# evan-wes/nerf-sandbox

Hardware: NVIDIA B200
Metric: train_rays_per_s (higher is better)
Workload: dtype bf16

## Files before the change

nerf_sandbox_b200/csrc/field_tc.cu:

```cuda
#include <cuda.h>
#include <cuda_bf16.h>
#include <cuda_fp16.h>
#include <cstdio>
#include <mutex>
#include "nsb_common.cuh"
#include "tc_ptx.cuh"

namespace nsb {
namespace tc {

constexpr int TILE_M = 128;
constexpr int kStageBytes = 16384;
constexpr int kStages = 4;
constexpr int kActBytes = TILE_M * 256 * 2;
constexpr int kGxBytes = TILE_M * 64 * 2;
constexpr int kSmemAct = 0;
constexpr int kSmemGx = 2 * kActBytes;
constexpr int kSmemRing = kSmemGx + 2 * kGxBytes;
constexpr int kSmemBar = kSmemRing + kStages * kStageBytes;
constexpr int kSmemBias = kSmemBar + 256;
constexpr int kSmemBytes = kSmemBias + 2048;
constexpr int kThreads = 384;
constexpr int kStages2 = 8;
constexpr int kStageBytes2 = kStageBytes / 2;
static_assert(8 * (3 * kStages2 + 6) + 4 <= 256, "barrier block overflow");
constexpr int kNumMmaLayers = 10;
constexpr uint32_t kTmemCols = 512;

__constant__ uint32_t c_layer_ofs[kNumMmaLayers] = {0,      32768,  163840, 294912, 425984,
                                                    589824, 720896, 851968, 983040, 1114112};
constexpr uint32_t kWeightImageBytes = 1114112 + 288 * 128 * 2;
constexpr uint32_t kBiasOfs = kWeightImageBytes;
constexpr int kBiasFloats = 9 * 256 + 128;
constexpr int kWsigOfs = kBiasFloats;
constexpr int kBsigOfs = kWsigOfs + 256;
constexpr int kWoOfs = kBsigOfs + 4;
constexpr int kBoOfs = kWoOfs + 384;
constexpr int kTailFloats = kBoOfs + 4;
constexpr uint32_t kTImgOfs = ((kBiasOfs + kTailFloats * 4 + 255) / 256) * 256;
constexpr int kNumDgradLayers = 9;
__host__ __device__ inline uint32_t dgrad_layer_ofs(int m) { return kTImgOfs + (m == 0 ? 0u : 65536u + (uint32_t)(m - 1) * 131072u); }
constexpr uint32_t kF16ImgOfs = kTImgOfs + 65536 + 8 * 131072;
static_assert(kF16ImgOfs % 256 == 0 && kWeightImageBytes % 256 == 0, "images are addressed as rows of 256 B");
constexpr uint32_t kF16LoImgOfs = kF16ImgOfs + kWeightImageBytes;
constexpr uint32_t kDinImgOfs = kF16LoImgOfs + kWeightImageBytes;
constexpr uint32_t kDinPos0 = 0, kDinPos4 = 32768, kDinDir = 65536, kDinImgBytes = 73728;
constexpr uint32_t kPackedTcBytes = kDinImgOfs + kDinImgBytes;

__host__ __device__ inline int layer_nslabs(int l) { return l == 0 ? 2 : (l == 4 ? 10 : (l == 9 ? 9 : 8)); }
__host__ __device__ inline int layer_N(int l) { return l == 9 ? 128 : 256; }
__host__ __device__ inline int layer_bias_ofs(int l) { return l * 256; }

constexpr uint32_t kFmtF16 = 0u, kFmtBF16 = 1u;
__device__ __forceinline__ uint32_t make_idesc2(int N, uint32_t a_fmt, uint32_t b_fmt) {
    return (1u << 4) | (a_fmt << 7) | (b_fmt << 10) | ((uint32_t)(N >> 3) << 17) | ((uint32_t)((2 * TILE_M) >> 4) << 24);
}

__device__ __forceinline__ uint32_t pack_bf16_relu(float a, float b) {
    uint32_t d;
    asm("cvt.rn.relu.bf16x2.f32 %0, %1, %2;" : "=r"(d) : "f"(b), "f"(a));
    return d;
}
__device__ __forceinline__ uint32_t pack_bf16(float a, float b) {
    __nv_bfloat162 t = __floats2bfloat162_rn(a, b);
    return *reinterpret_cast<uint32_t*>(&t);
}
__device__ __forceinline__ uint32_t pack_f16(float a, float b) {
    uint32_t d;
    asm("cvt.rn.satfinite.f16x2.f32 %0, %1, %2;" : "=r"(d) : "f"(b), "f"(a));
    return d;
}
__device__ __forceinline__ uint32_t pack_f16_relu(float a, float b) {
    uint32_t d;
    asm("cvt.rn.relu.satfinite.f16x2.f32 %0, %1, %2;" : "=r"(d) : "f"(b), "f"(a));
    return d;
}
template <bool F16> __device__ __forceinline__ uint32_t pack2(float a, float b) { return F16 ? pack_f16(a, b) : pack_bf16(a, b); }
template <bool F16> __device__ __forceinline__ uint32_t pack2_relu(float a, float b) { return F16 ? pack_f16_relu(a, b) : pack_bf16_relu(a, b); }

__device__ __forceinline__ uint32_t relu_bits16(const uint32_t (&w)[8]) {
    uint32_t s = 0;
#pragma unroll
    for (int j = 0; j < 8; ++j) s += __vsetne2(w[j], 0u) << j;
    return s;
}
__device__ __forceinline__ uint32_t relu_mask_word(uint32_t bits16, int j) { return ((bits16 >> j) & 0x00010001u) * 0xFFFFu; }

__device__ __forceinline__ void st_chunk(uint32_t base, int k8, int r, uint32_t a, uint32_t b, uint32_t c, uint32_t d);
__device__ __forceinline__ void st_chunk_g(uint8_t* grow, int k8, uint32_t a, uint32_t b, uint32_t c, uint32_t d);
__device__ __forceinline__ float4 lds_f4(uint32_t addr) {
    float4 v;
    asm volatile("ld.shared.v4.f32 {%0, %1, %2, %3}, [%4];" : "=f"(v.x), "=f"(v.y), "=f"(v.z), "=f"(v.w) : "r"(addr));
    return v;
}
template <int KIND, bool MASK>
__device__ __forceinline__ void epi_chunk16(const uint32_t (&v)[16], int c0, const float4 (&bias)[4], uint32_t act, int r, float& sig,
                                            float (&rgb)[3], float hw0, float hw1, float hw2, uint32_t& mbits) {
    float f[16];
#pragma unroll
    for (int j = 0; j < 4; ++j) {
        f[4 * j] = __uint_as_float(v[4 * j]) + bias[j].x; f[4 * j + 1] = __uint_as_float(v[4 * j + 1]) + bias[j].y;
        f[4 * j + 2] = __uint_as_float(v[4 * j + 2]) + bias[j].z; f[4 * j + 3] = __uint_as_float(v[4 * j + 3]) + bias[j].w;
    }
    if (KIND == 1 || KIND == 3) {
// ... 8 lines not shown
                rgb[2] = fmaf(f[j], __shfl_sync(0xffffffffu, hw2, src0 + j), rgb[2]);
            }
        }
    }
    if (KIND != 3 || MASK) {
        uint32_t w[8];
#pragma unroll
        for (int j = 0; j < 8; ++j) w[j] = KIND == 0 ? pack2_relu<!MASK>(f[2 * j], f[2 * j + 1]) : pack2<!MASK>(f[2 * j], f[2 * j + 1]);
        st_chunk(act, (c0 >> 3), r, w[0], w[1], w[2], w[3]);
        st_chunk(act, (c0 >> 3) + 1, r, w[4], w[5], w[6], w[7]);
        if (KIND != 2 && MASK) mbits = relu_bits16(w);
    }
}
template <int KIND, bool MASK>
__device__ __forceinline__ void epi_columns(uint32_t tmem_row, uint32_t sbias, uint32_t act, int r, int lane, const float* __restrict__ tail,
                                            float& sig, float (&rgb)[3], uint32_t* gmask) {
    constexpr int N = KIND == 3 ? 128 : 256;
    float hw0 = 0.f, hw1 = 0.f, hw2 = 0.f;
    if (KIND == 1) hw0 = __ldg(tail + kWsigOfs + lane);
    if (KIND == 3) { hw0 = __ldg(tail + kWoOfs + lane); hw1 = __ldg(tail + kWoOfs + 128 + lane); hw2 = __ldg(tail + kWoOfs + 256 + lane); }
    uint32_t mw[8] = {0u, 0u, 0u, 0u, 0u, 0u, 0u, 0u};
    uint32_t va[16], vb[16];
    tc_ld16(tmem_row, va);
#pragma unroll 1
    for (int c0 = 0; c0 < N; c0 += 32) {
        float4 ba[4], bb[4];
#pragma unroll
        for (int j = 0; j < 4; ++j) { ba[j] = lds_f4(sbias + 4u * (uint32_t)(c0 + 4 * j)); bb[j] = lds_f4(sbias + 4u * (uint32_t)(c0 + 16 + 4 * j)); }
        float n0 = 0.f, n1 = 0.f, n2 = 0.f;
        if (KIND == 1 && c0 + 32 < N) n0 = __ldg(tail + kWsigOfs + c0 + 32 + lane);
        if (KIND == 3 && c0 + 32 < N) {
            n0 = __ldg(tail + kWoOfs + c0 + 32 + lane); n1 = __ldg(tail + kWoOfs + 128 + c0 + 32 + lane);
            n2 = __ldg(tail + kWoOfs + 256 + c0 + 32 + lane);
        }
        tc_wait_ld();
        tc_ld16(tmem_row + (uint32_t)c0 + 16u, vb);
        pin16(va);
        uint32_t m0 = 0, m1 = 0;
        epi_chunk16<KIND, MASK>(va, c0, ba, act, r, sig, rgb, hw0, hw1, hw2, m0);
        tc_wait_ld();
        tc_ld16(tmem_row + (uint32_t)(c0 + 32 < N ? c0 + 32 : c0), va);
        pin16(vb);
        epi_chunk16<KIND, MASK>(vb, c0 + 16, bb, act, r, sig, rgb, hw0, hw1, hw2, m1);
        if (MASK) {
            const uint32_t m = m0 | (m1 << 8);
#pragma unroll
            for (int k = 0; k < 8; ++k) mw[k] = (c0 >> 5) == k ? m : mw[k];
        }
        hw0 = n0; hw1 = n1; hw2 = n2;
    }
    if (MASK && gmask) {
        reinterpret_cast<uint4*>(gmask)[0] = make_uint4(mw[0], mw[1], mw[2], mw[3]);
        reinterpret_cast<uint4*>(gmask)[1] = make_uint4(mw[4], mw[5], mw[6], mw[7]);
    }
}

struct FwdParams {
    const float* rays_o; const float* rays_d; const float* z; const float* ray_norm; const float* viewdirs;
    const float* enc_pos; const float* enc_dir;
    const uint8_t* packed;
    float* raw;
    uint8_t* stash;
    float* dbg; int dbg_layer;
    unsigned long long* cyc;
    int64_t Q; int N;
    int64_t num_tiles;
    alignas(64) CUtensorMap tm8;
    alignas(64) CUtensorMap tm4;
};

constexpr size_t kStashGx = 0, kStashH = 16384, kStashFeat = kStashH + 8 * 65536, kStashGd = kStashFeat + 65536,
                 kStashC = kStashGd + 8192,
                 kStashMask = kStashC + 32768, kStashTile = kStashMask + 9 * 128 * 32;
constexpr size_t kDstashTile = 32768 + 9 * 65536;
__host__ __device__ inline size_t dstash_ofs(int k) { return k == 9 ? 0 : 32768 + (size_t)(8 - k) * 65536; }

__device__ __forceinline__ void named_bar_sync(int id, int nthreads) {
    asm volatile("bar.sync %0, %1;" ::"r"(id), "r"(nthreads) : "memory");
}
__device__ __forceinline__ void named_bar_arrive(int id, int nthreads) {
    asm volatile("bar.arrive %0, %1;" ::"r"(id), "r"(nthreads) : "memory");
}
constexpr int kHandoffBar = 3;
__device__ __forceinline__ void handoff_signal(int t) {
    tc_fence_before();
    named_bar_arrive(kHandoffBar + t, 160);
}
__device__ __forceinline__ void handoff_wait(int t) {
    named_bar_sync(kHandoffBar + t, 160);
    tc_fence_after();
    fence_async_smem();
    tc_fence_before();
}
__device__ __forceinline__ void arrive_in(uint32_t crank, uint32_t bar_in, uint32_t bar_pin, int t) {
    if (crank == 0) mbar_arrive(bar_in + 8 * t); else mbar_arrive_remote(bar_pin + 8 * t, 0);
}
__device__ __forceinline__ void bulk_wait_all0() { asm volatile("cp.async.bulk.wait_group 0;" ::: "memory"); }

__device__ __forceinline__ void st_chunk(uint32_t base, int k8, int r, uint32_t a, uint32_t b, uint32_t c, uint32_t d) {
    asm volatile("st.shared.v4.b32 [%0], {%1, %2, %3, %4};" ::"r"(base + (uint32_t)k8 * 2048u + (uint32_t)r * 16u), "r"(a), "r"(b),
                 "r"(c), "r"(d)
                 : "memory");
}

__device__ __forceinline__ void st_chunk_g(uint8_t* grow, int k8, uint32_t a, uint32_t b, uint32_t c, uint32_t d) {
    if (grow) *reinterpret_cast<uint4*>(grow + (size_t)k8 * 2048) = make_uint4(a, b, c, d);
}

template <bool F16>
__device__ __forceinline__ void encode_pos(uint32_t gx, int r, float px, float py, float pz, uint8_t* grow) {
    float e[64];
    e[0] = px; e[1] = py; e[2] = pz; e[63] = 0.f;
    float s[3], c[3];
    sincosf(px, &s[0], &c[0]); sincosf(py, &s[1], &c[1]); sincosf(pz, &s[2], &c[2]);
#pragma unroll
    for (int k = 0; k < 10; ++k) {
#pragma unroll
        for (int d = 0; d < 3; ++d) {
            e[3 + 3 * k + d] = s[d]; e[33 + 3 * k + d] = c[d];
            const float s2 = 2.0f * s[d] * c[d], c2 = fmaf(-2.0f * s[d], s[d], 1.0f);
            s[d] = s2; c[d] = c2;
        }
    }
#pragma unroll
    for (int k8 = 0; k8 < 8; ++k8) {
        const uint32_t w0 = pack2<F16>(e[8 * k8], e[8 * k8 + 1]), w1 = pack2<F16>(e[8 * k8 + 2], e[8 * k8 + 3]),
                       w2 = pack2<F16>(e[8 * k8 + 4], e[8 * k8 + 5]), w3 = pack2<F16>(e[8 * k8 + 6], e[8 * k8 + 7]);
        st_chunk(gx, k8, r, w0, w1, w2, w3);
        st_chunk_g(grow, k8, w0, w1, w2, w3);
    }
}
template <bool F16>
__device__ __forceinline__ void encode_dir(uint32_t gx, int r, float vx, float vy, float vz, uint8_t* grow) {
    float e[32];
#pragma unroll
    for (int i = 27; i < 32; ++i) e[i] = 0.f;
    e[0] = vx; e[1] = vy; e[2] = vz;
    float s[3], c[3];
    sincosf(vx, &s[0], &c[0]); sincosf(vy, &s[1], &c[1]); sincosf(vz, &s[2], &c[2]);
#pragma unroll
    for (int k = 0; k < 4; ++k) {
#pragma unroll
        for (int d = 0; d < 3; ++d) {
            e[3 + 3 * k + d] = s[d]; e[15 + 3 * k + d] = c[d];
            const float s2 = 2.0f * s[d] * c[d], c2 = fmaf(-2.0f * s[d], s[d], 1.0f);
            s[d] = s2; c[d] = c2;
        }
    }
#pragma unroll
    for (int k8 = 0; k8 < 4; ++k8) {
        const uint32_t w0 = pack2<F16>(e[8 * k8], e[8 * k8 + 1]), w1 = pack2<F16>(e[8 * k8 + 2], e[8 * k8 + 3]),
                       w2 = pack2<F16>(e[8 * k8 + 4], e[8 * k8 + 5]), w3 = pack2<F16>(e[8 * k8 + 6], e[8 * k8 + 7]);
        st_chunk(gx, k8, r, w0, w1, w2, w3);
        st_chunk_g(grow, k8, w0, w1, w2, w3);
    }
}
template <bool F16>
__device__ __forceinline__ void copy_enc_row(uint32_t gx, int r, const float* __restrict__ src, int n, int chunks, uint8_t* grow) {
    for (int k8 = 0; k8 < chunks; ++k8) {
        float v[8];
#pragma unroll
        for (int j = 0; j < 8; ++j) v[j] = (8 * k8 + j < n && src) ? src[8 * k8 + j] : 0.f;
        const uint32_t w0 = pack2<F16>(v[0], v[1]), w1 = pack2<F16>(v[2], v[3]), w2 = pack2<F16>(v[4], v[5]), w3 = pack2<F16>(v[6], v[7]);
        st_chunk(gx, k8, r, w0, w1, w2, w3);
        st_chunk_g(grow, k8, w0, w1, w2, w3);
    }
// ... 531 lines not shown
    }
    tc_fence_before();
    __syncthreads();
    cluster_sync_all();
    if (warp == 2) {
        tc_fence_after();
        asm volatile("tcgen05.dealloc.cta_group::2.sync.aligned.b32 %0, %1;" ::"r"(tmem_base), "r"(kTmemCols) : "memory");
    }
}

__device__ __forceinline__ float f16_residual(float x) {
    const __half h = __float2half_rn(fminf(fmaxf(x, -65504.0f), 65504.0f));
    return (x - __half2float(h)) * 2048.0f;
}
template <int FMT>
__device__ __forceinline__ void pack_tc_forward(const float* __restrict__ params, uint8_t* __restrict__ out, int m) {
    constexpr bool F16 = FMT != 0;
    {
        const int pl = m < 9 ? m : 10;
        const LayerDesc d = layer_desc(pl);
        const int N = d.N, Kp = d.Kpad;
        __nv_bfloat16* img = reinterpret_cast<__nv_bfloat16*>(out + (FMT == 2 ? kF16LoImgOfs : FMT == 1 ? kF16ImgOfs : 0u) + c_layer_ofs[m]);
        const int hn = N >> 1;
        for (int idx = blockIdx.x * blockDim.x + threadIdx.x; idx < N * (Kp >> 3); idx += gridDim.x * blockDim.x) {
            const int k8 = idx / N, n = idx % N;
            const float* row = params + d.w_off + (int64_t)n * d.K + 8 * k8;
            uint32_t w[4];
#pragma unroll
            for (int j = 0; j < 4; ++j) {
                float a = 8 * k8 + 2 * j < d.K ? row[2 * j] : 0.f, b = 8 * k8 + 2 * j + 1 < d.K ? row[2 * j + 1] : 0.f;
                if (FMT == 2) { a = f16_residual(a); b = f16_residual(b); }
                w[j] = pack2<F16>(a, b);
            }
            reinterpret_cast<uint4*>(img)[(((size_t)(k8 >> 2) * 2 + n / hn) * 4 + (k8 & 3)) * hn + n % hn] = make_uint4(w[0], w[1], w[2], w[3]);
        }
        if (FMT != 0) return;
        float* tail = reinterpret_cast<float*>(out + kBiasOfs);
        for (int n = blockIdx.x * blockDim.x + threadIdx.x; n < N; n += gridDim.x * blockDim.x)
            tail[layer_bias_ofs(m) + n] = params[d.b_off + n];
    }
    if (m == 0) {
        float* tail = reinterpret_cast<float*>(out + kBiasOfs);
        const LayerDesc ds = layer_desc(9), dc = layer_desc(11);
        for (int i = blockIdx.x * blockDim.x + threadIdx.x; i < 256; i += gridDim.x * blockDim.x) tail[kWsigOfs + i] = params[ds.w_off + i];
        for (int i = blockIdx.x * blockDim.x + threadIdx.x; i < 384; i += gridDim.x * blockDim.x) tail[kWoOfs + i] = params[dc.w_off + i];
        if (blockIdx.x == 0 && threadIdx.x < 4) {
            tail[kBsigOfs + threadIdx.x] = threadIdx.x == 0 ? params[ds.b_off] : 0.f;
            tail[kBoOfs + threadIdx.x] = threadIdx.x < 3 ? params[dc.b_off + threadIdx.x] : 0.f;
        }
    }
}

struct DgradParams {
    const float* d_raw;
    const uint8_t* packed;
    const uint8_t* stash;
    uint8_t* dstash;
    int64_t Q; int64_t num_tiles;
    alignas(64) CUtensorMap tm8;
};

__device__ __forceinline__ uint4 ldg16(const uint8_t* p) { return __ldg(reinterpret_cast<const uint4*>(p)); }
__device__ __forceinline__ float bf16lo(uint32_t w) { return __uint_as_float(w << 16); }
__device__ __forceinline__ float bf16hi(uint32_t w) { return __uint_as_float(w & 0xffff0000u); }

template <int KIND>
__device__ __forceinline__ void dgrad_chunk16(const uint32_t (&v)[16], int c0, uint32_t act, int r, float dsig, float hw0, uint32_t bits16) {
    uint32_t w[8];
#pragma unroll
    for (int j = 0; j < 8; ++j) {
        float a = __uint_as_float(v[2 * j]), b = __uint_as_float(v[2 * j + 1]);
        if (KIND == 1) {
            a = fmaf(dsig, __shfl_sync(0xffffffffu, hw0, (c0 & 16) + 2 * j), a);
            b = fmaf(dsig, __shfl_sync(0xffffffffu, hw0, (c0 & 16) + 2 * j + 1), b);
        }
        w[j] = pack_bf16(a, b);
        if (KIND != 0) w[j] &= relu_mask_word(bits16, j);
    }
    st_chunk(act, (c0 >> 3), r, w[0], w[1], w[2], w[3]);
    st_chunk(act, (c0 >> 3) + 1, r, w[4], w[5], w[6], w[7]);
}
template <int KIND>
__device__ __forceinline__ void dgrad_columns(uint32_t tmem_row, uint32_t act, int r, int lane, const float* __restrict__ tail,
                                              const uint4& mlo, const uint4& mhi, float dsig) {
    float hw0 = KIND == 1 ? __ldg(tail + kWsigOfs + lane) : 0.f;
    const uint32_t mw[8] = {mlo.x, mlo.y, mlo.z, mlo.w, mhi.x, mhi.y, mhi.z, mhi.w};
    uint32_t va[16], vb[16];
    tc_ld16(tmem_row, va);
#pragma unroll
    for (int i = 0; i < 8; ++i) {
        const int c0 = 32 * i;
        float n0 = 0.f;
        if (KIND == 1 && i < 7) n0 = __ldg(tail + kWsigOfs + c0 + 32 + lane);
        tc_wait_ld();
        tc_ld16(tmem_row + (uint32_t)c0 + 16u, vb);
        pin16(va);
        dgrad_chunk16<KIND>(va, c0, act, r, dsig, hw0, mw[i]);
        tc_wait_ld();
        tc_ld16(tmem_row + (uint32_t)(i < 7 ? c0 + 32 : c0), va);
        pin16(vb);
        dgrad_chunk16<KIND>(vb, c0 + 16, act, r, dsig, hw0, mw[i] >> 8);
        hw0 = n0;
    }
}

constexpr int kDgStages = 12;
constexpr int kDgSmemRing = kSmemGx;
static_assert(kDgSmemRing + kDgStages * kStageBytes2 == kSmemBar, "dgrad ring must end at the barrier block");
static_assert(kSmemBar + 8 * (3 * kDgStages + 6) + 4 <= kSmemBytes, "barrier block overflow");
__global__ void __cluster_dims__(2, 1, 1) __launch_bounds__(kThreads, 1) field_dgrad_kernel(const __grid_constant__ DgradParams p) {
    extern __shared__ __align__(128) uint8_t smem[];
    const uint32_t sbase = smem_u32(smem);
    const int warp = threadIdx.x >> 5, lane = threadIdx.x & 31;
    const uint32_t crank = cluster_ctarank();
    const uint32_t bar_full = sbase + kSmemBar, bar_empty = bar_full + 8 * kDgStages, bar_in = bar_empty + 8 * kDgStages,
                   bar_acc = bar_in + 16, bar_pfull = bar_acc + 16, bar_pin = bar_pfull + 8 * kDgStages;
    volatile uint32_t* tmem_slot = reinterpret_cast<volatile uint32_t*>(smem + kSmemBar + 8 * (3 * kDgStages + 6));
    if (threadIdx.x == 0) {
        for (int s = 0; s < kDgStages; ++s) { mbar_init(bar_full + 8 * s, 1); mbar_init(bar_empty + 8 * s, 1); mbar_init(bar_pfull + 8 * s, 1); }
        for (int t = 0; t < 2; ++t) { mbar_init(bar_in + 8 * t, 1); mbar_init(bar_acc + 8 * t, 1); mbar_init(bar_pin + 8 * t, 1); }
        asm volatile("fence.mbarrier_init.release.cluster;" ::: "memory");
    }
    if (warp == 2) {
        asm volatile("tcgen05.alloc.cta_group::2.sync.aligned.shared::cta.b32 [%0], %1;" ::"r"(smem_u32((const void*)tmem_slot)),
                     "r"(kTmemCols)
                     : "memory");
        asm volatile("tcgen05.relinquish_alloc_permit.cta_group::2.sync.aligned;" ::: "memory");
    }
    tc_fence_before();
    __syncthreads();
    cluster_sync_all();
    tc_fence_after();
    const uint32_t tmem_base = *tmem_slot;
    const int64_t num_pairs = (p.num_tiles + 1) / 2;
    const int64_t first_pair = (int64_t)blockIdx.x - crank;
    const int64_t n_iter = first_pair < num_pairs ? (num_pairs - first_pair + gridDim.x - 1) / gridDim.x : 0;
    const float* tail = reinterpret_cast<const float*>(p.packed + kBiasOfs);

    if (warp == 0) {
        {
            uint32_t stage = 0, round = 0;
            for (int64_t it = 0, pair = blockIdx.x; it < n_iter; ++it, pair += gridDim.x) {
                for (int m = 0; m < kNumDgradLayers; ++m) {
                    const uint8_t* src = p.packed + dgrad_layer_ofs(m);
                    const int ns = m == 0 ? 4 : 8;
                    for (int s = 0; s < ns; ++s) {
                        mbar_wait(bar_empty + 8 * stage, (round & 1) ^ 1);
                        if (elect_one()) {
                            if (crank == 0) mbar_expect_tx(bar_full + 8 * stage, kStageBytes);
                            tma_load_rows_to_leader(sbase + kDgSmemRing + stage * kStageBytes2, &p.tm8,
                                                    (dgrad_layer_ofs(m) + (uint32_t)s * kStageBytes + crank * kStageBytes2) >> 8, bar_full + 8 * stage);
                        }
                        __syncwarp();
                        if (++stage == kDgStages) { stage = 0; ++round; }
                    }
                }
            }
        }
    } else if (warp == 1) {
        if (crank == 0 && elect_one()) {
            uint32_t stage = 0, round = 0, use = 0;
            const uint32_t idesc = make_idesc2(256, kFmtBF16, kFmtBF16);
            const uint64_t ahi = desc_hi(2048, 128), bhi = desc_hi(2048, 128);
            const uint32_t ring_lo = (sbase + kDgSmemRing) >> 4;
            for (int64_t it = 0; it < n_iter; ++it) {
                for (int m = 0; m < kNumDgradLayers; ++m, ++use) {
                    const int ns = m == 0 ? 4 : 8;
                    const uint32_t stage0 = stage, round0 = round;
                    for (int t = 0; t < 2; ++t) {
                        mbar_wait(bar_in + 8 * t, use & 1);
                        mbar_wait_cl(bar_pin + 8 * t, use & 1);
                        tc_fence_after();
                        if (t == 1) { stage = stage0; round = round0; }
                        const uint32_t d_tmem = tmem_base + (uint32_t)t * 256u;
                        uint32_t a_lo = (sbase + kSmemAct + t * kActBytes) >> 4;
                        for (int s = 0; s < ns; ++s, a_lo += 512u) {
                            if (t == 0) {
                                mbar_wait(bar_full + 8 * stage, round & 1);
                                tc_fence_after();
                            }
                            const uint32_t b_lo = ring_lo + stage * (kStageBytes2 >> 4);
                            tc_mma2(d_tmem, ahi | (uint64_t)a_lo, bhi | (uint64_t)b_lo, idesc, s > 0 ? 1u : 0u);
                            tc_mma2(d_tmem, ahi | (uint64_t)(a_lo + 256u), bhi | (uint64_t)(b_lo + 256u), idesc, 1u);
                            if (s == ns - 1) tc_commit2(bar_acc + 8 * t);
                            if (t == 1) tc_commit2(bar_empty + 8 * stage);
                            if (++stage == kDgStages) { stage = 0; ++round; }
                        }
                    }
                }
            }
        }
    } else if (warp == 2 || warp == 3) {
        const int t = warp - 2;
        const uint32_t act = sbase + kSmemAct + t * kActBytes;
        named_bar_arrive(1 + t, 160);
        for (int64_t it = 0, pair = blockIdx.x; it < n_iter; ++it, pair += gridDim.x) {
            const int64_t tile = pair * 2 + t;
            uint8_t* ds_tile = tile < p.num_tiles ? p.dstash + (size_t)tile * kDstashTile : nullptr;
            const bool last_pair = it + 1 == n_iter;
            for (int e = 0; e <= kNumDgradLayers; ++e) {
                handoff_wait(t);
                if (lane == 0) {
                    if (e < kNumDgradLayers) arrive_in(crank, bar_in, bar_pin, t);
                    if (ds_tile) {
                        bulk_s2g(ds_tile + (e == 0 ? dstash_ofs(9) : dstash_ofs(8 - (e - 1))), act, e == 0 ? 32768u : 65536u);
                        bulk_commit();
                        bulk_wait_read0();
                    }
                }
                __syncwarp();
                if (!(last_pair && e == kNumDgradLayers)) named_bar_arrive(1 + t, 160);
            }
        }
        if (lane == 0) bulk_wait_all0();
    } else if (warp >= 4) {
        const int t = (warp - 4) >> 2;
        const int r = (int)threadIdx.x - 128 - t * 128;
        const uint32_t act = sbase + kSmemAct + t * kActBytes;
        const uint32_t tmem_row = tmem_base + (uint32_t)t * 256u + ((uint32_t)((warp & 3) * 32) << 16);
        uint32_t use = 0;
        for (int64_t it = 0, pair = blockIdx.x; it < n_iter; ++it, pair += gridDim.x) {
            const int64_t tile = pair * 2 + t;
            const int64_t q = tile * TILE_M + r;
            const bool tile_ok = tile < p.num_tiles;
            const bool valid = tile_ok && q < p.Q;
            const uint8_t* st_tile = p.stash + (size_t)(tile_ok ? tile : 0) * kStashTile;
            const float4 d = valid ? __ldg(reinterpret_cast<const float4*>(p.d_raw) + q) : make_float4(0.f, 0.f, 0.f, 0.f);
            named_bar_sync(1 + t, 160);
            {
                const uint8_t* mrow = st_tile + kStashMask + (size_t)r * 32;
                const uint4 cbits = ldg16(mrow + 8 * 4096);
                const uint32_t cw[4] = {cbits.x, cbits.y, cbits.z, cbits.w};
#pragma unroll
                for (int g = 0; g < 4; ++g) {
                    const float w0 = __ldg(tail + kWoOfs + 32 * g + lane), w1 = __ldg(tail + kWoOfs + 128 + 32 * g + lane),
                                w2 = __ldg(tail + kWoOfs + 256 + 32 * g + lane);
#pragma unroll
                    for (int c8 = 0; c8 < 4; ++c8) {
                        const uint32_t bits16 = cw[g] >> (8 * (c8 >> 1));
                        uint32_t w[4];
#pragma unroll
                        for (int j2 = 0; j2 < 4; ++j2) {
                            const int s0 = c8 * 8 + 2 * j2;
                            const float ga = d.x * __shfl_sync(0xffffffffu, w0, s0) + d.y * __shfl_sync(0xffffffffu, w1, s0) +
                                             d.z * __shfl_sync(0xffffffffu, w2, s0);
                            const float gb = d.x * __shfl_sync(0xffffffffu, w0, s0 + 1) + d.y * __shfl_sync(0xffffffffu, w1, s0 + 1) +
                                             d.z * __shfl_sync(0xffffffffu, w2, s0 + 1);
                            w[j2] = pack_bf16(ga, gb) & relu_mask_word(bits16, 4 * (c8 & 1) + j2);
                        }
                        st_chunk(act, g * 4 + c8, r, w[0], w[1], w[2], w[3]);
                    }
                }
            }
            handoff_signal(t);
            for (int m = 0; m < kNumDgradLayers; ++m, ++use) {
                uint4 mlo = make_uint4(0, 0, 0, 0), mhi = mlo;
                if (m >= 1) {
                    const uint8_t* mrow = st_tile + kStashMask + (size_t)(8 - m) * 4096 + (size_t)r * 32;
                    mlo = ldg16(mrow); mhi = ldg16(mrow + 16);
                }
                mbar_wait(bar_acc + 8 * t, use & 1);
                tc_fence_after();
                named_bar_sync(1 + t, 160);
                if (m == 0) dgrad_columns<0>(tmem_row, act, r, lane, tail, mlo, mhi, d.w);
                else if (m == 1) dgrad_columns<1>(tmem_row, act, r, lane, tail, mlo, mhi, d.w);
                else dgrad_columns<2>(tmem_row, act, r, lane, tail, mlo, mhi, d.w);
                handoff_signal(t);
            }
        }
    }
    tc_fence_before();
    __syncthreads();
    cluster_sync_all();
    if (warp == 2) {
        tc_fence_after();
        asm volatile("tcgen05.dealloc.cta_group::2.sync.aligned.b32 %0, %1;" ::"r"(tmem_base), "r"(kTmemCols) : "memory");
    }
}

struct WgPiece { uint32_t ofs; uint32_t bytes; int from_stash; int dy_half; int head; };
struct WgGroup { int a_piece, b_piece, b_piece2, tmem_col, n; };
enum { HEAD_NONE = 0, HEAD_SIGMA = 1, HEAD_RGB = 2 };
struct WgradJob {
    int n_pieces; WgPiece pieces[4];
    int n_groups; WgGroup groups[4];
    int release_after[4];
    int halves, xcols;
    int64_t w_dst;
    int ldw;
    int ncols_valid;
    int64_t b_dst;
    int64_t head_w_dst, head_b_dst;
    int cta_begin, cta_count;
};
constexpr int kMaxJobs = 16;
struct WgradParams {
    const uint8_t* stash; const uint8_t* dstash; const float* d_raw; float* grads;
    int64_t num_tiles, Q; int num_jobs; int dbg;
    WgradJob jobs[kMaxJobs];
};
constexpr int kWgPiece = 32768;
constexpr int kWgSlots = 6;
constexpr int kWgSmemBar = kWgSlots * kWgPiece;
constexpr int kWgSmemBytes = kWgSmemBar + 256;
constexpr int kWgThreads = 256;

__device__ __forceinline__ uint32_t make_idesc_mn(int N) {
    return (1u << 4) | (kFmtBF16 << 7) | (kFmtBF16 << 10) | (1u << 15) | (1u << 16) | ((uint32_t)(N >> 3) << 17) | ((uint32_t)(TILE_M >> 4) << 24);
}

template <int KIND>
__device__ __forceinline__ void wg_colsum(const uint8_t* img, int nchunks, int w4, int lane, const float4 (&dr)[4], float (&a0)[4][8],
                                          float (&a1)[4][8], float (&a2)[4][8]) {
#pragma unroll
    for (int ii = 0; ii < 4; ++ii) {
        const int c8 = w4 + 4 * ii;
        if (c8 < nchunks) {
#pragma unroll
            for (int rg = 0; rg < 4; ++rg) {
                const uint4 v = *reinterpret_cast<const uint4*>(img + (size_t)c8 * 2048 + (size_t)(rg * 32 + lane) * 16);
                const float x[8] = {bf16lo(v.x), bf16hi(v.x), bf16lo(v.y), bf16hi(v.y), bf16lo(v.z), bf16hi(v.z), bf16lo(v.w), bf16hi(v.w)};
#pragma unroll
                for (int j = 0; j < 8; ++j) {
                    if (KIND == 0) a0[ii][j] += x[j];
                    else if (KIND == 1) a0[ii][j] = fmaf(dr[rg].w, x[j], a0[ii][j]);
                    else {
                        a0[ii][j] = fmaf(dr[rg].x, x[j], a0[ii][j]); a1[ii][j] = fmaf(dr[rg].y, x[j], a1[ii][j]);
                        a2[ii][j] = fmaf(dr[rg].z, x[j], a2[ii][j]);
                    }
                }
            }
        }
    }
}

__global__ void __launch_bounds__(kWgThreads, 1) field_wgrad_kernel(const __grid_constant__ WgradParams p) {
    extern __shared__ __align__(128) uint8_t smem[];
    const uint32_t sbase = smem_u32(smem);
    const int warp = threadIdx.x >> 5, lane = threadIdx.x & 31;
    const uint32_t bar_full = sbase + kWgSmemBar, bar_empty = bar_full + 8 * kWgSlots, bar_done = bar_empty + 8 * kWgSlots;
    volatile uint32_t* tmem_slot = reinterpret_cast<volatile uint32_t*>(smem + kWgSmemBar + 8 * (2 * kWgSlots + 2));
    int ji = 0;
    for (int j = 0; j < p.num_jobs; ++j)
        if ((int)blockIdx.x >= p.jobs[j].cta_begin && (int)blockIdx.x < p.jobs[j].cta_begin + p.jobs[j].cta_count) ji = j;
    const WgradJob& job = p.jobs[ji];
    const int part = (int)blockIdx.x - job.cta_begin;
    if (threadIdx.x == 0) {
        for (int s = 0; s < kWgSlots; ++s) { mbar_init(bar_full + 8 * s, 1); mbar_init(bar_empty + 8 * s, 1 + 4); }
        mbar_init(bar_done, 1);
        asm volatile("fence.mbarrier_init.release.cluster;" ::: "memory");
// ... 439 lines not shown

template <bool FROM_ENC>
static int launch_fwd(tc::FwdParams& p, cudaStream_t st) {
    NSB_TRY(check_arch());
    static bool attr_set = false;
    if (!attr_set) {
        if (cudaFuncSetAttribute(tc::field_fwd_kernel<FROM_ENC, false>, cudaFuncAttributeMaxDynamicSharedMemorySize, tc::kSmemBytes) != cudaSuccess ||
            cudaFuncSetAttribute(tc::field_fwd_kernel<FROM_ENC, true>, cudaFuncAttributeMaxDynamicSharedMemorySize, tc::kSmemBytes) != cudaSuccess)
            return check_launch("cudaFuncSetAttribute(field_fwd_kernel)");
        attr_set = true;
    }
    p.num_tiles = cdiv(p.Q, tc::TILE_M);
    NSB_TRY(packed_maps(p.packed, &p.tm8, &p.tm4));
    const int64_t pairs = (p.num_tiles + 1) / 2;
    int grid = (int)(pairs < num_sms() ? pairs : num_sms());
    grid = (grid + 1) / 2 * 2;
    if (grid > num_sms()) grid -= 2;
    if (p.stash) tc::field_fwd_kernel<FROM_ENC, true><<<grid, tc::kThreads, tc::kSmemBytes, st>>>(p);
    else tc::field_fwd_kernel<FROM_ENC, false><<<grid, tc::kThreads, tc::kSmemBytes, st>>>(p);
    NSB_LAUNCH_CHECK("field_fwd_kernel");
    return NSB_OK;
}

template <bool FROM_ENC>
static int launch_fwd_split(tc::FwdParams& p, cudaStream_t st) {
    NSB_TRY(check_arch());
    static bool attr_set = false;
    if (!attr_set) {
        if (cudaFuncSetAttribute(tc::field_fwd_split_kernel<FROM_ENC>, cudaFuncAttributeMaxDynamicSharedMemorySize, tc::kSmemBytes) != cudaSuccess)
            return check_launch("cudaFuncSetAttribute(field_fwd_split_kernel)");
        attr_set = true;
    }
    p.num_tiles = cdiv(p.Q, tc::TILE_M);
    NSB_TRY(packed_maps(p.packed, &p.tm8, &p.tm4));
    const int64_t pairs = (p.num_tiles + 1) / 2;
    const int64_t max_pairs = num_sms() / 2;
    const int grid = 2 * (int)(pairs < max_pairs ? pairs : max_pairs);
    tc::field_fwd_split_kernel<FROM_ENC><<<grid, tc::kThreads, tc::kSmemBytes, st>>>(p);
    NSB_LAUNCH_CHECK("field_fwd_split_kernel");
    return NSB_OK;
}

int tc_field_fwd_rays_split(const float* rays_o, const float* rays_d, const float* z, const float* ray_norm, const float* viewdirs,
                            const void* packed, float* raw, int64_t B, int N, cudaStream_t st) {
    tc::FwdParams p{};
    p.rays_o = rays_o; p.rays_d = rays_d; p.z = z; p.ray_norm = ray_norm; p.viewdirs = viewdirs;
    p.packed = reinterpret_cast<const uint8_t*>(packed); p.raw = raw;
    p.Q = B * (int64_t)N; p.N = N;
    return launch_fwd_split<false>(p, st);
}
int tc_field_fwd_enc_split(const float* enc_pos, const float* enc_dir, const void* packed, float* raw, int64_t Q, cudaStream_t st) {
    tc::FwdParams p{};
    p.enc_pos = enc_pos; p.enc_dir = enc_dir;
    p.packed = reinterpret_cast<const uint8_t*>(packed); p.raw = raw;
    p.Q = Q; p.N = 1;
    return launch_fwd_split<true>(p, st);
}

int tc_field_fwd_rays(const float* rays_o, const float* rays_d, const float* z, const float* ray_norm, const float* viewdirs,
                      const void* packed, float* raw, void* ws, int64_t B, int N, int stash, cudaStream_t st) {
    tc::FwdParams p{};
    p.rays_o = rays_o; p.rays_d = rays_d; p.z = z; p.ray_norm = ray_norm; p.viewdirs = viewdirs;
    p.packed = reinterpret_cast<const uint8_t*>(packed); p.raw = raw;
    p.stash = stash ? ws_stash(ws) : nullptr;
    p.Q = B * (int64_t)N; p.N = N;
    return launch_fwd<false>(p, st);
}

int tc_field_fwd_enc(const float* enc_pos, const float* enc_dir, const void* packed, float* raw, void* ws, int64_t Q,
                     int stash, cudaStream_t st) {
    tc::FwdParams p{};
    p.enc_pos = enc_pos; p.enc_dir = enc_dir;
    p.packed = reinterpret_cast<const uint8_t*>(packed); p.raw = raw;
    p.stash = stash ? ws_stash(ws) : nullptr;
    p.Q = Q; p.N = 1;
    return launch_fwd<true>(p, st);
}

int tc_field_bwd(const float* d_raw, const void* packed, float* grads, float* d_enc_pos, float* d_enc_dir, void* ws, int64_t Q,
                 cudaStream_t st) {
    NSB_TRY(check_arch());
    static bool attr_set = false;
    if (!attr_set) {
        if (cudaFuncSetAttribute(tc::field_dgrad_kernel, cudaFuncAttributeMaxDynamicSharedMemorySize, tc::kSmemBytes) != cudaSuccess ||
            cudaFuncSetAttribute(tc::field_wgrad_kernel, cudaFuncAttributeMaxDynamicSharedMemorySize, tc::kWgSmemBytes) != cudaSuccess ||
            cudaFuncSetAttribute(tc::field_dinput_kernel, cudaFuncAttributeMaxDynamicSharedMemorySize, tc::kDiSmemBytes) != cudaSuccess)
            return check_launch("cudaFuncSetAttribute(bwd kernels)");
        attr_set = true;
    }
    const int64_t tiles = cdiv(Q, tc::TILE_M);
    const int64_t pairs = (tiles + 1) / 2;
    tc::DgradParams dp{};
    dp.d_raw = d_raw; dp.packed = reinterpret_cast<const uint8_t*>(packed); dp.stash = ws_stash(ws); dp.dstash = ws_dstash(ws, Q);
    dp.Q = Q; dp.num_tiles = tiles;
    NSB_TRY(packed_maps(packed, &dp.tm8, nullptr));
    int dgrid = (int)(pairs < num_sms() ? pairs : num_sms());
    dgrid = (dgrid + 1) / 2 * 2;
    if (dgrid > num_sms()) dgrid -= 2;
    tc::field_dgrad_kernel<<<dgrid, tc::kThreads, tc::kSmemBytes, st>>>(dp);
    NSB_LAUNCH_CHECK("field_dgrad_kernel");
    if (d_enc_pos || d_enc_dir) {
        tc::DinputParams ip{};
        ip.packed = reinterpret_cast<const uint8_t*>(packed); ip.dstash = ws_dstash(ws, Q);
        ip.d_enc_pos = d_enc_pos; ip.d_enc_dir = d_enc_dir; ip.Q = Q; ip.num_tiles = tiles;
        const int igrid = (int)(tiles < num_sms() ? tiles : num_sms());
        tc::field_dinput_kernel<<<igrid, tc::kDiThreads, tc::kDiSmemBytes, st>>>(ip);
        NSB_LAUNCH_CHECK("field_dinput_kernel");
    }
    if (!grads) return NSB_OK;

    tc::WgradParams wp{};
    wp.stash = ws_stash(ws); wp.dstash = ws_dstash(ws, Q); wp.d_raw = d_raw; wp.grads = grads; wp.num_tiles = tiles; wp.Q = Q;
    int nj = 0;
    auto add = [&](int k, size_t x_ofs, int xcols, int pl, int col0, int valid, bool bias, int head) {
        const LayerDesc d = layer_desc(pl);
        tc::WgradJob& j = wp.jobs[nj++];
        j = tc::WgradJob{};
        const int halves = k == 9 ? 1 : 2;
        const uint32_t dy = (uint32_t)tc::dstash_ofs(k);
        const uint32_t xb = (uint32_t)xcols * 256u;
        auto piece = [&](uint32_t ofs, uint32_t bytes, int from_stash, int dy_half, int hd) {
            j.pieces[j.n_pieces] = tc::WgPiece{ofs, bytes, from_stash, dy_half, hd}; j.release_after[j.n_pieces] = -1; return j.n_pieces++;
        };
        auto group = [&](int a, int b, int col, int n) {
            j.groups[j.n_groups] = tc::WgGroup{a, b, -1, col, n}; j.release_after[a] = j.n_groups; j.release_after[b] = j.n_groups; ++j.n_groups;
        };
        if (xcols == 256) {
            const int b0 = piece((uint32_t)x_ofs, 32768, 1, -1, head), b1 = piece((uint32_t)x_ofs + 32768, 32768, 1, -1, head);
            const int a0 = piece(dy, 32768, 0, 0, 0);
            group(a0, b0, 0, 256);
            if (halves == 2) { const int a1 = piece(dy + 32768, 32768, 0, 1, 0); group(a1, b0, 256, 256); }
            for (int g = 0; g < j.n_groups; ++g) j.groups[g].b_piece2 = b1;
            j.release_after[b1] = j.n_groups - 1;
        } else {
            const int a0 = piece(dy, 32768, 0, 0, 0);
            const int b0 = piece((uint32_t)x_ofs, xb, 1, -1, head);
            group(a0, b0, 0, xcols);
            if (halves == 2) { const int a1 = piece(dy + 32768, 32768, 0, 1, 0); group(a1, b0, 256, xcols); }
        }
        j.halves = halves; j.xcols = xcols;
        j.w_dst = d.w_off + col0; j.ldw = d.K; j.ncols_valid = valid; j.b_dst = bias ? d.b_off : -1;
        if (head == tc::HEAD_SIGMA) { const LayerDesc ds = layer_desc(9); j.head_w_dst = ds.w_off; j.head_b_dst = ds.b_off; }
    };
    add(0, tc::kStashGx, 64, 0, 0, 63, true, 0);
    for (int l = 1; l <= 7; ++l) {
        add(l, tc::kStashH + (size_t)(l - 1) * 65536, 256, l, 0, 256, true, 0);
        if (l == 4) add(4, tc::kStashGx, 64, 4, 256, 63, false, 0);
    }
    add(8, tc::kStashH + 7 * 65536, 256, 8, 0, 256, true, tc::HEAD_SIGMA);
    add(9, tc::kStashFeat, 256, 10, 0, 256, true, 0);
    add(9, tc::kStashGd, 32, 10, 256, 27, false, 0);
    {
        tc::WgradJob& j = wp.jobs[nj++];
        j = tc::WgradJob{};
        j.pieces[0] = tc::WgPiece{(uint32_t)tc::kStashC, 32768, 1, -1, tc::HEAD_RGB}; j.release_after[0] = -1; j.n_pieces = 1;
        const LayerDesc dc = layer_desc(11);
        j.head_w_dst = dc.w_off; j.head_b_dst = dc.b_off; j.b_dst = -1;
    }
    wp.num_jobs = nj;
    wp.dbg = getenv("NSB_WG_DBG") != nullptr;
    const int total = num_sms();
    double cost[tc::kMaxJobs];
    for (int i = 0; i < nj; ++i) {
        const tc::WgradJob& j = wp.jobs[i];
        if (j.n_groups == 0) cost[i] = 1750;
        else if (j.xcols == 256) cost[i] = j.halves == 2 ? 5600 : 3100;
        else cost[i] = j.xcols == 64 ? 3750 : 2100;
        if (j.head_w_dst && j.n_groups) cost[i] += 100;
        wp.jobs[i].cta_count = 1;
    }
    for (int used = nj; used < total; ++used) {
        int worst = -1; double worst_t = -1;
        for (int i = 0; i < nj; ++i) {
            if ((int64_t)wp.jobs[i].cta_count >= tiles) continue;
            const double t = cost[i] * (double)cdiv(tiles, wp.jobs[i].cta_count);
            if (t > worst_t) { worst_t = t; worst = i; }
        }
        if (worst < 0) break;
        ++wp.jobs[worst].cta_count;
    }
    int begin = 0;
    for (int i = 0; i < nj; ++i) { wp.jobs[i].cta_begin = begin; begin += wp.jobs[i].cta_count; }
// ... 21 lines not shown
```

Before: 814,300.

## Pipeline dgrad activation handoff per quarter with mbarriers instead of named barriers

Replaces the whole-tile named-barrier handoff between the epilogue warps and the copy/issue warp with per-quarter mbarriers. Each 16KB quarter of the activation buffer is copied to the dstash via bulk copy as soon as it is written, and is released back once its read completes. The goal is to overlap the epilogue's TMEM-to-smem writes with the global stash stores and the next MMA arrival, at the cost of extra mbarrier traffic and more complex parity tracking.

```diff
diff --git a/nerf_sandbox_b200/csrc/field_tc.cu b/nerf_sandbox_b200/csrc/field_tc.cu
--- a/nerf_sandbox_b200/csrc/field_tc.cu
+++ b/nerf_sandbox_b200/csrc/field_tc.cu
@@ -20,6 +20,9 @@
 constexpr int kSmemBar = kSmemRing + kStages * kStageBytes;
 constexpr int kSmemBias = kSmemBar + 256;
 constexpr int kSmemBytes = kSmemBias + 2048;
+constexpr int kSmemQbar = kSmemBytes;
+constexpr int kSmemDgradBytes = kSmemQbar + 2 * 8 * 8;
+static_assert(kSmemDgradBytes <= 232448, "227 KB of shared memory per block");
 constexpr int kThreads = 384;
 constexpr int kStages2 = 8;
 constexpr int kStageBytes2 = kStageBytes / 2;
@@ -194,6 +197,41 @@
     asm volatile("bar.arrive %0, %1;" ::"r"(id), "r"(nthreads) : "memory");
 }
 constexpr int kHandoffBar = 3;
+constexpr int kQuarterBytes = 16384;
+__device__ __forceinline__ uint32_t quarter_bars(uint32_t sbase, int t) { return sbase + kSmemQbar + 64u * (uint32_t)t; }
+__device__ __forceinline__ void quarter_bars_init(uint32_t sbase) {
+    for (int t = 0; t < 2; ++t)
+        for (int q = 0; q < 4; ++q) { mbar_init(quarter_bars(sbase, t) + 8 * q, 4); mbar_init(quarter_bars(sbase, t) + 32 + 8 * q, 1); }
+}
+__device__ __forceinline__ void quarter_acquire(uint32_t qbar, int q, uint32_t par) {
+    const uint32_t bar = qbar + 32 + 8 * (uint32_t)q, parity = ((par >> q) & 1u) ^ 1u;
+    while (!mbar_try_wait(bar, parity)) {}
+}
+__device__ __forceinline__ void quarter_written(uint32_t qbar, int q, uint32_t& par, int lane) {
+    __syncwarp();
+    if (lane == 0) mbar_arrive(qbar + 8 * (uint32_t)q);
+    par ^= 1u << q;
+}
+__device__ __forceinline__ void quarter_wait(uint32_t qbar, int q, uint32_t& par) {
+    mbar_wait(qbar + 8 * (uint32_t)q, (par >> q) & 1u);
+    par ^= 1u << q;
+    tc_fence_after();
+    fence_async_smem();
+    tc_fence_before();
+}
+__device__ __forceinline__ void quarters_release(uint32_t qbar, int nq, bool copied) {
+    for (int q = 0; q < nq; ++q) {
+        if (copied) {
+            switch (nq - 1 - q) {
+                case 3: asm volatile("cp.async.bulk.wait_group.read 3;" ::: "memory"); break;
+                case 2: asm volatile("cp.async.bulk.wait_group.read 2;" ::: "memory"); break;
+                case 1: asm volatile("cp.async.bulk.wait_group.read 1;" ::: "memory"); break;
+                default: asm volatile("cp.async.bulk.wait_group.read 0;" ::: "memory"); break;
+            }
+        }
+        mbar_arrive(qbar + 32 + 8 * (uint32_t)q);
+    }
+}
 __device__ __forceinline__ void handoff_signal(int t) {
     tc_fence_before();
     named_bar_arrive(kHandoffBar + t, 160);
@@ -891,7 +929,7 @@
 }
 template <int KIND>
 __device__ __forceinline__ void dgrad_columns(uint32_t tmem_row, uint32_t act, int r, int lane, const float* __restrict__ tail,
-                                              const uint4& mlo, const uint4& mhi, float dsig) {
+                                              const uint4& mlo, const uint4& mhi, float dsig, uint32_t qbar, uint32_t& qpar) {
     float hw0 = KIND == 1 ? __ldg(tail + kWsigOfs + lane) : 0.f;
     const uint32_t mw[8] = {mlo.x, mlo.y, mlo.z, mlo.w, mhi.x, mhi.y, mhi.z, mhi.w};
     uint32_t va[16], vb[16];
@@ -904,11 +942,13 @@
         tc_wait_ld();
         tc_ld16(tmem_row + (uint32_t)c0 + 16u, vb);
         pin16(va);
+        if ((i & 1) == 0) quarter_acquire(qbar, i >> 1, qpar);
         dgrad_chunk16<KIND>(va, c0, act, r, dsig, hw0, mw[i]);
         tc_wait_ld();
         tc_ld16(tmem_row + (uint32_t)(i < 7 ? c0 + 32 : c0), va);
         pin16(vb);
         dgrad_chunk16<KIND>(vb, c0 + 16, act, r, dsig, hw0, mw[i] >> 8);
+        if ((i & 1) == 1 && i < 7) quarter_written(qbar, i >> 1, qpar, lane);
         hw0 = n0;
     }
 }
@@ -928,6 +968,7 @@
     if (threadIdx.x == 0) {
         for (int s = 0; s < kDgStages; ++s) { mbar_init(bar_full + 8 * s, 1); mbar_init(bar_empty + 8 * s, 1); mbar_init(bar_pfull + 8 * s, 1); }
         for (int t = 0; t < 2; ++t) { mbar_init(bar_in + 8 * t, 1); mbar_init(bar_acc + 8 * t, 1); mbar_init(bar_pin + 8 * t, 1); }
+        quarter_bars_init(sbase);
         asm volatile("fence.mbarrier_init.release.cluster;" ::: "memory");
     }
     if (warp == 2) {
@@ -1001,33 +1042,36 @@
         }
     } else if (warp == 2 || warp == 3) {
         const int t = warp - 2;
-        const uint32_t act = sbase + kSmemAct + t * kActBytes;
-        named_bar_arrive(1 + t, 160);
-        for (int64_t it = 0, pair = blockIdx.x; it < n_iter; ++it, pair += gridDim.x) {
-            const int64_t tile = pair * 2 + t;
-            uint8_t* ds_tile = tile < p.num_tiles ? p.dstash + (size_t)tile * kDstashTile : nullptr;
-            const bool last_pair = it + 1 == n_iter;
-            for (int e = 0; e <= kNumDgradLayers; ++e) {
-                handoff_wait(t);
-                if (lane == 0) {
-                    if (e < kNumDgradLayers) arrive_in(crank, bar_in, bar_pin, t);
-                    if (ds_tile) {
-                        bulk_s2g(ds_tile + (e == 0 ? dstash_ofs(9) : dstash_ofs(8 - (e - 1))), act, e == 0 ? 32768u : 65536u);
-                        bulk_commit();
-                        bulk_wait_read0();
-                    }
-                }
-                __syncwarp();
-                if (!(last_pair && e == kNumDgradLayers)) named_bar_arrive(1 + t, 160);
-            }
-        }
-        if (lane == 0) bulk_wait_all0();
+        const uint32_t act = sbase + kSmemAct + t * kActBytes, qbar = quarter_bars(sbase, t);
+        if (lane == 0) {
+            uint32_t qpar = 0;
+            for (int64_t it = 0, pair = blockIdx.x; it < n_iter; ++it, pair += gridDim.x) {
+                const int64_t tile = pair * 2 + t;
+                uint8_t* ds_tile = tile < p.num_tiles ? p.dstash + (size_t)tile * kDstashTile : nullptr;
+                for (int e = 0; e <= kNumDgradLayers; ++e) {
+                    const int nq = e == 0 ? 2 : 4;
+                    uint8_t* dst = ds_tile ? ds_tile + (e == 0 ? dstash_ofs(9) : dstash_ofs(8 - (e - 1))) : nullptr;
+                    for (int q = 0; q < nq; ++q) {
+                        quarter_wait(qbar, q, qpar);
+                        if (q == nq - 1 && e < kNumDgradLayers) arrive_in(crank, bar_in, bar_pin, t);
+                        if (dst) {
+                            bulk_s2g(dst + (size_t)q * kQuarterBytes, act + (uint32_t)q * kQuarterBytes, kQuarterBytes);
+                            bulk_commit();
+                        }
+                    }
+                    quarters_release(qbar, nq, dst != nullptr);
+                }
+            }
+            bulk_wait_all0();
+        }
+        __syncwarp();
     } else if (warp >= 4) {
         const int t = (warp - 4) >> 2;
         const int r = (int)threadIdx.x - 128 - t * 128;
         const uint32_t act = sbase + kSmemAct + t * kActBytes;
         const uint32_t tmem_row = tmem_base + (uint32_t)t * 256u + ((uint32_t)((warp & 3) * 32) << 16);
-        uint32_t use = 0;
+        const uint32_t qbar = quarter_bars(sbase, t);
+        uint32_t use = 0, qpar = 0;
         for (int64_t it = 0, pair = blockIdx.x; it < n_iter; ++it, pair += gridDim.x) {
             const int64_t tile = pair * 2 + t;
             const int64_t q = tile * TILE_M + r;
@@ -1035,7 +1079,6 @@
             const bool valid = tile_ok && q < p.Q;
             const uint8_t* st_tile = p.stash + (size_t)(tile_ok ? tile : 0) * kStashTile;
             const float4 d = valid ? __ldg(reinterpret_cast<const float4*>(p.d_raw) + q) : make_float4(0.f, 0.f, 0.f, 0.f);
-            named_bar_sync(1 + t, 160);
             {
                 const uint8_t* mrow = st_tile + kStashMask + (size_t)r * 32;
                 const uint4 cbits = ldg16(mrow + 8 * 4096);
@@ -1044,6 +1087,7 @@
                 for (int g = 0; g < 4; ++g) {
                     const float w0 = __ldg(tail + kWoOfs + 32 * g + lane), w1 = __ldg(tail + kWoOfs + 128 + 32 * g + lane),
                                 w2 = __ldg(tail + kWoOfs + 256 + 32 * g + lane);
+                    if ((g & 1) == 0) quarter_acquire(qbar, g >> 1, qpar);
 #pragma unroll
                     for (int c8 = 0; c8 < 4; ++c8) {
                         const uint32_t bits16 = cw[g] >> (8 * (c8 >> 1));
@@ -1059,9 +1103,11 @@
                         }
                         st_chunk(act, g * 4 + c8, r, w[0], w[1], w[2], w[3]);
                     }
-                }
-            }
-            handoff_signal(t);
+                    if (g == 1) quarter_written(qbar, 0, qpar, lane);
+                }
+            }
+            tc_fence_before();
+            quarter_written(qbar, 1, qpar, lane);
             for (int m = 0; m < kNumDgradLayers; ++m, ++use) {
                 uint4 mlo = make_uint4(0, 0, 0, 0), mhi = mlo;
                 if (m >= 1) {
@@ -1070,11 +1116,11 @@
                 }
                 mbar_wait(bar_acc + 8 * t, use & 1);
                 tc_fence_after();
-                named_bar_sync(1 + t, 160);
-                if (m == 0) dgrad_columns<0>(tmem_row, act, r, lane, tail, mlo, mhi, d.w);
-                else if (m == 1) dgrad_columns<1>(tmem_row, act, r, lane, tail, mlo, mhi, d.w);
-                else dgrad_columns<2>(tmem_row, act, r, lane, tail, mlo, mhi, d.w);
-                handoff_signal(t);
+                if (m == 0) dgrad_columns<0>(tmem_row, act, r, lane, tail, mlo, mhi, d.w, qbar, qpar);
+                else if (m == 1) dgrad_columns<1>(tmem_row, act, r, lane, tail, mlo, mhi, d.w, qbar, qpar);
+                else dgrad_columns<2>(tmem_row, act, r, lane, tail, mlo, mhi, d.w, qbar, qpar);
+                tc_fence_before();
+                quarter_written(qbar, 3, qpar, lane);
             }
         }
     }
@@ -1680,7 +1726,7 @@
     NSB_TRY(check_arch());
     static bool attr_set = false;
     if (!attr_set) {
-        if (cudaFuncSetAttribute(tc::field_dgrad_kernel, cudaFuncAttributeMaxDynamicSharedMemorySize, tc::kSmemBytes) != cudaSuccess ||
+        if (cudaFuncSetAttribute(tc::field_dgrad_kernel, cudaFuncAttributeMaxDynamicSharedMemorySize, tc::kSmemDgradBytes) != cudaSuccess ||
             cudaFuncSetAttribute(tc::field_wgrad_kernel, cudaFuncAttributeMaxDynamicSharedMemorySize, tc::kWgSmemBytes) != cudaSuccess ||
             cudaFuncSetAttribute(tc::field_dinput_kernel, cudaFuncAttributeMaxDynamicSharedMemorySize, tc::kDiSmemBytes) != cudaSuccess)
             return check_launch("cudaFuncSetAttribute(bwd kernels)");
@@ -1695,7 +1741,7 @@
     int dgrid = (int)(pairs < num_sms() ? pairs : num_sms());
     dgrid = (dgrid + 1) / 2 * 2;
     if (dgrid > num_sms()) dgrid -= 2;
-    tc::field_dgrad_kernel<<<dgrid, tc::kThreads, tc::kSmemBytes, st>>>(dp);
+    tc::field_dgrad_kernel<<<dgrid, tc::kThreads, tc::kSmemDgradBytes, st>>>(dp);
     NSB_LAUNCH_CHECK("field_dgrad_kernel");
     if (d_enc_pos || d_enc_dir) {
         tc::DinputParams ip{};
```

Result: no change. 812,800 (median of 6 runs) (-0.2%).
